# yangdongchao/Text-to-sound-Synthesis

Measured on NVIDIA H100. Metric: clips/sec (10s audio, 100 diffusion steps), higher is better.
Workload: dtype f16x3

## Files before the change

include/diffsound_b200.h:

```cpp
#ifndef DIFFSOUND_B200_H
#define DIFFSOUND_B200_H

#include <stdint.h>

#ifdef __cplusplus
extern "C" {
#endif

#define DSB_VERSION 100

#define DSB_DTYPE_TF32 0
#define DSB_DTYPE_BF16 1
#define DSB_DTYPE_F16 2

#define DSB_GEMM_GELU2 1
#define DSB_GEMM_ROUND_TF32 2
#define DSB_GEMM_OUT_BF16 4
#define DSB_GEMM_LRELU 8
#define DSB_GEMM_TANH 16
#define DSB_GEMM_OUT_F16 256
#define DSB_GEMM_RES_BEFORE_ACT 128
#define DSB_GEMM_DUAL_LRELU 4096
#define DSB_GEMM_NO_STORE 16384
#define DSB_GEMM_OUT_F16_SPLIT 2048
// ... 22 lines not shown
  int num_taps;
  int tap_shift[32];
  int tap_acol[32];
  long long a_cols;
  int geo_P, geo_Wp, geo_y0, geo_y1, geo_x0, geo_x1;
  float alpha;
  int block_n;
  int max_ctas;
  int cta_pair;
  int a_mn_major;
  int b_mn_major;
  int use_tap_wcol;
  int tap_wcol[32];
  long long w_cols;
  long long split_off;
  long long dual_off;
  int out_col_group;
  int out_col_group_stride;
  const void* A2;
  long long a2_rows, a2_cols, lda2, a2_batch_stride;
  int tap_a2[32];
  float* amax_out;
  int resident_w;
} dsb_gemm_desc;
int dsb_gemm_ex(const dsb_gemm_desc* desc, void* stream);

int dsb_gemm_f32(const float* A, const float* W, const float* bias, const float* residual, float* out, int M, int N, int K,
                 long long lda, long long ldw, long long ldo, long long ld_res, int flags, void* stream);

int dsb_round_tf32(const float* in, float* out, long long n, void* stream);
int dsb_f32_to_bf16(const float* in, void* out_bf16, long long n, void* stream);
int dsb_f32_to_f16(const float* in, void* out_f16, long long n, void* stream);
int dsb_split_f16(const float* in, long long ld_in, void* out_f16, long long ld_out, long long lo_off, long long rows, int C, float scale,
                  void* stream);
int dsb_split_tf32(const float* in, long long ld_in, float* out, long long ld_out, long long rows, int C, int Cp, int w_format, void* stream);

int dsb_embed_tokens(const int64_t* ids, const float* emb, const float* height_emb, const float* width_emb, float* out, int B, int L,
                     int D, int H, int W, int num_embed, int* err_flag, void* stream);

int dsb_layernorm(const float* x, void* out, const float* gamma, const float* beta, int rows, int D, float eps, int flags, void* stream);

int dsb_ada_layernorm(const float* x, void* out, const float* table, const int64_t* t, int B, int L, int D, int T, float eps, int flags,
                      void* stream);

int dsb_l2_normalize_rows(float* x, long long rows, int D, void* stream);

// ... 87 lines not shown
```

text-to-sound-synthesis_b200/_lib.py:

```python
from __future__ import annotations

import ctypes as C
import os

_HERE = os.path.dirname(os.path.abspath(__file__))
LIB_PATH = os.path.join(_HERE, "libdiffsound_b200.so")

c_vp, c_i, c_ll, c_f = C.c_void_p, C.c_int, C.c_longlong, C.c_float


class GemmDesc(C.Structure):
    _fields_ = [
        ("A", c_vp), ("W", c_vp), ("bias", c_vp), ("residual", c_vp), ("out", c_vp),
        ("M", c_i), ("N", c_i), ("K", c_i), ("batch", c_i),
        ("a_rows", c_ll), ("lda", c_ll), ("ldw", c_ll), ("ldo", c_ll), ("ld_res", c_ll),
        ("a_batch_stride", c_ll), ("w_batch_stride", c_ll), ("out_batch_stride", c_ll), ("res_batch_stride", c_ll),
        ("dtype", c_i), ("flags", c_i), ("num_taps", c_i), ("tap_shift", c_i * 32), ("tap_acol", c_i * 32), ("a_cols", c_ll),
        ("geo_P", c_i), ("geo_Wp", c_i), ("geo_y0", c_i), ("geo_y1", c_i), ("geo_x0", c_i), ("geo_x1", c_i),
        ("alpha", c_f), ("block_n", c_i), ("max_ctas", c_i), ("cta_pair", c_i), ("a_mn_major", c_i), ("b_mn_major", c_i),
        ("use_tap_wcol", c_i), ("tap_wcol", c_i * 32), ("w_cols", c_ll), ("split_off", c_ll),
        ("dual_off", c_ll), ("out_col_group", c_i), ("out_col_group_stride", c_i), ("A2", c_vp),
        ("a2_rows", c_ll), ("a2_cols", c_ll), ("lda2", c_ll), ("a2_batch_stride", c_ll), ("tap_a2", c_i * 32), ("amax_out", c_vp), ("resident_w", c_i),
    ]


SIGNATURES = {
    "dsb_version": [],
    "dsb_device_info": [C.POINTER(c_i)] * 3,
    "dsb_gemm_ex": [C.POINTER(GemmDesc), c_vp],
    "dsb_gemm_f32": [c_vp] * 5 + [c_i] * 3 + [c_ll] * 4 + [c_i, c_vp],
    "dsb_round_tf32": [c_vp, c_vp, c_ll, c_vp],
    "dsb_f32_to_bf16": [c_vp, c_vp, c_ll, c_vp],
    "dsb_f32_to_f16": [c_vp, c_vp, c_ll, c_vp],
    "dsb_silu": [c_vp, c_vp, c_ll, c_vp],
    "dsb_split_f16": [c_vp, c_ll, c_vp, c_ll, c_ll, c_ll, c_i, c_f, c_vp],
    "dsb_attention_tc_split": [c_vp, c_ll, c_ll, c_vp, c_ll, c_ll, c_vp, c_ll, c_ll, c_vp, c_ll, c_ll, c_i, c_i, c_i, c_i, c_f, c_vp],
    "dsb_l2_normalize_rows": [c_vp, c_ll, c_i, c_vp],
    "dsb_split_tf32": [c_vp, c_ll, c_vp, c_ll, c_ll, c_i, c_i, c_i, c_vp],
    "dsb_embed_tokens": [c_vp] * 5 + [c_i] * 6 + [c_vp, c_vp],
    "dsb_layernorm": [c_vp] * 4 + [c_i, c_i, c_f, c_i, c_vp],
    "dsb_ada_layernorm": [c_vp] * 4 + [c_i] * 4 + [c_f, c_i, c_vp],
    "dsb_attention": [c_vp, c_ll, c_vp, c_ll, c_vp, c_ll, c_vp, c_ll, c_i, c_i, c_i, c_i, c_f, c_i, c_vp],
    "dsb_codebook_gather_padded": [c_vp] * 3 + [c_i] * 6 + [c_vp, c_vp],
    "dsb_groupnorm_stats": [c_vp, c_vp] + [c_i] * 4 + [c_vp],
    "dsb_groupnorm_apply": [c_vp] * 5 + [c_i] * 5 + [c_f, c_i, c_i, c_vp],
# ... 60 lines not shown
```

text-to-sound-synthesis_b200/csrc/common.cuh:

```cuda
#pragma once
#include <cuda_runtime.h>
#include <cuda.h>
#include <cstdint>
#include <cstdio>

namespace dsb {

void set_error(const char* fmt, ...);
#define DSB_CHECK_CUDA(expr)                                                                    \
  do {                                                                                          \
    cudaError_t _e = (expr);                                                                    \
    if (_e != cudaSuccess) {                                                                    \
      dsb::set_error("%s:%d: %s -> %s", __FILE__, __LINE__, #expr, cudaGetErrorString(_e));     \
      return 1;                                                                                 \
    }                                                                                           \
  } while (0)
#define DSB_REQUIRE(cond, ...)                                                                  \
  do {                                                                                          \
    if (!(cond)) {                                                                              \
      dsb::set_error(__VA_ARGS__);                                                              \
      return 2;                                                                                 \
    }                                                                                           \
  } while (0)

// ... 59 lines not shown
__device__ __forceinline__ bool mbar_try_wait(uint64_t* bar, uint32_t parity) {
  uint32_t ok;
  asm volatile(
      "{\n\t.reg .pred P;\n\t"
      "mbarrier.try_wait.parity.shared::cta.b64 P, [%1], %2;\n\t"
      "selp.u32 %0, 1, 0, P;\n\t}"
      : "=r"(ok)
      : "r"(smem_u32(bar)), "r"(parity)
      : "memory");
  return ok != 0;
}
__device__ __forceinline__ void mbar_wait(uint64_t* bar, uint32_t parity) {
  uint32_t spins = 0;
  while (!mbar_try_wait(bar, parity)) {
    if (++spins > (1u << 26)) {
#ifdef DSB_MBAR_DEBUG
      printf("dsb: mbarrier wait timeout (block %d thread %d)\n", blockIdx.x, threadIdx.x);
#endif
      __trap();
    }
  }
}

__device__ __forceinline__ void prefetch_tmap(const CUtensorMap* m) {
  asm volatile("prefetch.tensormap [%0];" ::"l"(reinterpret_cast<uint64_t>(m)) : "memory");
}
__device__ __forceinline__ void tma_load_3d(const CUtensorMap* m, uint64_t* bar, void* dst, int c0, int c1, int c2) {
  asm volatile(
      "cp.async.bulk.tensor.3d.shared::cluster.global.mbarrier::complete_tx::bytes [%0], [%1, {%3, %4, %5}], [%2];"
      ::"r"(smem_u32(dst)), "l"(reinterpret_cast<uint64_t>(m)), "r"(smem_u32(bar)), "r"(c0), "r"(c1), "r"(c2)
      : "memory");
}

__device__ __forceinline__ void wgmma_fence() { asm volatile("wgmma.fence.sync.aligned;" ::: "memory"); }
__device__ __forceinline__ void wgmma_commit() { asm volatile("wgmma.commit_group.sync.aligned;" ::: "memory"); }
template <int N>
__device__ __forceinline__ void wgmma_wait() { asm volatile("wgmma.wait_group.sync.aligned %0;" ::"n"(N) : "memory"); }
template <int N>
__device__ __forceinline__ void wgmma_fence_regs(float (&d)[N]) {
#pragma unroll
  for (int i = 0; i < N; ++i) asm volatile("" : "+f"(d[i])::"memory");
}
template <uint32_t R>
__device__ __forceinline__ void setmaxnreg_inc() { asm volatile("setmaxnreg.inc.sync.aligned.u32 %0;" ::"n"(R)); }
template <uint32_t R>
__device__ __forceinline__ void setmaxnreg_dec() { asm volatile("setmaxnreg.dec.sync.aligned.u32 %0;" ::"n"(R)); }
// ... 13 lines not shown
```

text-to-sound-synthesis_b200/csrc/gemm_wgmma.cu:

```cuda
#include "common.cuh"
#include "diffsound_b200.h"
#include "wgmma.cuh"
#include <cuda_bf16.h>
#include <cuda_fp16.h>
#include <cstdlib>
#include <type_traits>

namespace dsb {

constexpr int BLOCK_M = 128;
constexpr int ROW_BYTES = 128;
constexpr int GEMM_THREADS = 384;
constexpr int MAX_TAPS = 32;
constexpr int MN_BOX_BYTES = 64 * ROW_BYTES;
constexpr int EPI_ROWS = 16;
constexpr int SMEM_BUDGET = 192 * 1024;

struct GemmParams {
  int M, N, batch;
  int tiles_m, tiles_n;
  int kb_per_tap;
  int block_k;
  int num_taps;
  int tap_shift[MAX_TAPS];
  int tap_acol[MAX_TAPS];
  int tap_wcol[MAX_TAPS];
  unsigned tap_a2_mask;
  int f3_nsp, lo_a, lo_w;
  long long split_off;
  long long dual_off;
  int ocg, ocg_stride;
  float* amax_out;
  int kc;
  int b_batched;
  const float* bias;
  const float* residual;
  long long ld_res, res_bstride;
  void* out;
  long long ldo, out_bstride;
  int flags;
  int geo_P, geo_Wp, geo_y0, geo_y1, geo_x0, geo_x1;
  float alpha;
  int a_mn, b_mn;
};

template <int BLOCK_N, bool F3>
struct GemmSmem {
  static constexpr int A_BYTES = BLOCK_M * ROW_BYTES;
  static constexpr int B_BYTES = BLOCK_N * ROW_BYTES;
  static constexpr int STAGE_BYTES = (F3 ? 2 : 1) * (A_BYTES + B_BYTES);
  static constexpr int STAGES = SMEM_BUDGET / STAGE_BYTES;
  static constexpr int EPI_BYTES = 8 * EPI_ROWS * 32 * 4;
  static constexpr int TOTAL = STAGES * STAGE_BYTES + EPI_BYTES + 256  + 1024 ;
};

__device__ __forceinline__ void epilogue_chunk(const GemmParams& p, const float* sw, int row_base, int col0, int b, int lane, bool vec_ok) {
  const bool has_geo = p.geo_P > 0;
  const int out_mode = (p.flags & DSB_GEMM_OUT_F16_SPLIT) ? 3 : ((p.flags & DSB_GEMM_OUT_F16) ? 1 : ((p.flags & DSB_GEMM_OUT_BF16) ? 2 : 0));
  const int act = (p.flags & DSB_GEMM_GELU2) ? 1 : ((p.flags & DSB_GEMM_LRELU) ? 2 : ((p.flags & DSB_GEMM_TANH) ? 3 : 0));
  const bool do_round = (p.flags & DSB_GEMM_ROUND_TF32) != 0;
  const bool dual = (p.flags & DSB_GEMM_DUAL_LRELU) != 0;
  const bool res_first = (p.flags & DSB_GEMM_RES_BEFORE_ACT) != 0;
  const int c4 = lane & 7;
  const int rsub = lane >> 3;
  constexpr int NI = EPI_ROWS / 4;
  uint32_t ok_mask = 0, in_mask = 0;
#pragma unroll
// ... 183 lines not shown
      }
    }
  }
}

template <int BLOCK_N, int KIND, bool F3>
__global__ void __launch_bounds__(GEMM_THREADS, 1)
gemm_wgmma_kernel(const __grid_constant__ CUtensorMap tmap_a, const __grid_constant__ CUtensorMap tmap_a2, const __grid_constant__ CUtensorMap tmap_b,
                  const __grid_constant__ GemmParams p) {
  using S = GemmSmem<BLOCK_N, F3>;
  constexpr int STAGES = S::STAGES;
  constexpr int NH = BLOCK_N / 128;
  static_assert(!F3 || NH == 1, "the split-fp16 form runs 128-wide tiles");
  extern __shared__ uint8_t smem_raw[];
  uint8_t* smem = reinterpret_cast<uint8_t*>((reinterpret_cast<uintptr_t>(smem_raw) + 1023) & ~uintptr_t(1023));
  float* epi_smem = reinterpret_cast<float*>(smem + STAGES * S::STAGE_BYTES);
  uint64_t* full_bar = reinterpret_cast<uint64_t*>(smem + STAGES * S::STAGE_BYTES + S::EPI_BYTES);
  uint64_t* empty_bar = full_bar + STAGES;

  const int warp = threadIdx.x >> 5;
  const int lane = threadIdx.x & 31;
  const int num_tiles = p.tiles_m * p.tiles_n * p.batch;
  const int num_kb = F3 ? p.kb_per_tap * p.f3_nsp : p.kb_per_tap * p.num_taps;

  if (threadIdx.x == 0) {
    prefetch_tmap(&tmap_a);
    prefetch_tmap(&tmap_a2);
    prefetch_tmap(&tmap_b);
    for (int s = 0; s < STAGES; ++s) {
      mbar_init(&full_bar[s], 1);
      mbar_init(&empty_bar[s], 8);
    }
    fence_barrier_init();
  }
  __syncthreads();
  pdl_wait();
  pdl_trigger();

  if (warp < 4) {
    setmaxnreg_dec<40>();
    if (threadIdx.x == 0) {
      int stage = 0;
      uint32_t phase = 0;
      for (int tile = blockIdx.x; tile < num_tiles; tile += gridDim.x) {
        const int m_blk = tile % p.tiles_m;
        const int n_blk = (tile / p.tiles_m) % p.tiles_n;
        const int b = tile / (p.tiles_m * p.tiles_n);
        for (int kb = 0; kb < num_kb; ++kb) {
          const int tap = kb / p.kb_per_tap;
          const int c0 = (kb - tap * p.kb_per_tap) * p.block_k;
          mbar_wait(&empty_bar[stage], phase ^ 1);
          mbar_arrive_expect_tx(&full_bar[stage], S::STAGE_BYTES);
          uint8_t* sa = smem + stage * S::STAGE_BYTES;
          if constexpr (F3) {
            const int arow = m_blk * BLOCK_M + p.tap_shift[tap], acol = p.tap_acol[tap] + c0, wcol = p.tap_wcol[tap] + c0;
            tma_load_3d(&tmap_a, &full_bar[stage], sa, acol, arow, b);
            tma_load_3d(&tmap_a, &full_bar[stage], sa + S::A_BYTES, acol + p.lo_a, arow, b);
            tma_load_3d(&tmap_b, &full_bar[stage], sa + 2 * S::A_BYTES, wcol, n_blk * BLOCK_N, 0);
            tma_load_3d(&tmap_b, &full_bar[stage], sa + 2 * S::A_BYTES + S::B_BYTES, wcol + p.lo_w, n_blk * BLOCK_N, 0);
          } else {
            if (p.a_mn) {
#pragma unroll
              for (int j = 0; j < BLOCK_M / 64; ++j) tma_load_3d(&tmap_a, &full_bar[stage], sa + j * MN_BOX_BYTES, m_blk * BLOCK_M + j * 64, c0, b);
            } else {
              tma_load_3d(((p.tap_a2_mask >> tap) & 1u) ? &tmap_a2 : &tmap_a, &full_bar[stage], sa, c0 + p.tap_acol[tap], m_blk * BLOCK_M + p.tap_shift[tap], b);
            }
            if (p.b_mn) {
#pragma unroll
              for (int j = 0; j < BLOCK_N / 64; ++j)
                tma_load_3d(&tmap_b, &full_bar[stage], sa + S::A_BYTES + j * MN_BOX_BYTES, n_blk * BLOCK_N + j * 64, c0, p.b_batched ? b : 0);
            } else {
              tma_load_3d(&tmap_b, &full_bar[stage], sa + S::A_BYTES, p.tap_wcol[tap] + c0, n_blk * BLOCK_N, p.b_batched ? b : 0);
            }
          }
          if (++stage == STAGES) { stage = 0; phase ^= 1; }
        }
      }
    }
  } else {
    setmaxnreg_inc<232>();
    const int wg = (warp >> 2) - 1;
    const int wq = warp & 3;
    float* sw = epi_smem + (warp - 4) * (EPI_ROWS * 32);
    const bool vec_ok = ((p.ldo & 3) == 0) && ((p.out_bstride & 3) == 0) && ((p.split_off & 3) == 0) && ((p.dual_off & 3) == 0) && ((p.ocg & 3) == 0) &&
                        ((p.ocg_stride & 3) == 0) &&
                        ((reinterpret_cast<uintptr_t>(p.out) & (4 * ((p.flags & (DSB_GEMM_OUT_F16_SPLIT | DSB_GEMM_OUT_F16 | DSB_GEMM_OUT_BF16)) ? 2 : 4) - 1)) == 0) &&
                        (!p.residual || (((p.ld_res & 3) == 0) && ((p.res_bstride & 3) == 0) && ((reinterpret_cast<uintptr_t>(p.residual) & 15) == 0))) &&
                        (!p.bias || ((reinterpret_cast<uintptr_t>(p.bias) & 15) == 0));
    int stage = 0;
    uint32_t phase = 0;
    for (int tile = blockIdx.x; tile < num_tiles; tile += gridDim.x) {
      const int m_blk = tile % p.tiles_m;
      const int n_blk = (tile / p.tiles_m) % p.tiles_n;
      const int b = tile / (p.tiles_m * p.tiles_n);
      float acc[NH][64];
#pragma unroll
      for (int h = 0; h < NH; ++h)
#pragma unroll
        for (int i = 0; i < 64; ++i) acc[h][i] = 0.f;
      int prev_stage = -1;
      if constexpr (F3) {
        float part[64];
        for (int kb = 0; kb < num_kb; ++kb) {
          mbar_wait(&full_bar[stage], phase);
          const uint32_t sa = smem_u32(smem + stage * S::STAGE_BYTES);
          wgmma_fence_regs(part);
          wgmma_fence();
          float(&pp)[1][64] = *reinterpret_cast<float(*)[1][64]>(&part);
          mma_kblock<KIND, 0, 0, 1, true>(pp, sa, wg, 0);
          wgmma_commit();
          wgmma_wait<0>();
          wgmma_fence_regs(part);
          if (lane == 0) mbar_arrive(&empty_bar[stage]);
#pragma unroll
          for (int i = 0; i < 64; ++i) acc[0][i] += part[i];
          if (++stage == STAGES) { stage = 0; phase ^= 1; }
        }
      } else {
        auto mainloop = [&](auto ta, auto tb) {
          for (int kb = 0; kb < num_kb; ++kb) {
            mbar_wait(&full_bar[stage], phase);
            const uint32_t sa = smem_u32(smem + stage * S::STAGE_BYTES);
#pragma unroll
            for (int h = 0; h < NH; ++h) wgmma_fence_regs(acc[h]);
            wgmma_fence();
            mma_kblock<KIND, decltype(ta)::value, decltype(tb)::value, NH, false>(acc, sa, wg, kb);
            wgmma_commit();
#pragma unroll
            for (int h = 0; h < NH; ++h) wgmma_fence_regs(acc[h]);
            wgmma_wait<1>();
            if (prev_stage >= 0 && lane == 0) mbar_arrive(&empty_bar[prev_stage]);
            prev_stage = stage;
            if (++stage == STAGES) { stage = 0; phase ^= 1; }
          }
        };
        using K0 = std::integral_constant<int, 0>;
        using K1 = std::integral_constant<int, 1>;
        if constexpr (KIND == DSB_DTYPE_TF32) mainloop(K0{}, K0{});
        else if (!p.a_mn && !p.b_mn) mainloop(K0{}, K0{});
        else if (p.a_mn && !p.b_mn) mainloop(K1{}, K0{});
        else if (!p.a_mn) mainloop(K0{}, K1{});
        else mainloop(K1{}, K1{});
      }
      wgmma_wait<0>();
#pragma unroll
      for (int h = 0; h < NH; ++h) wgmma_fence_regs(acc[h]);
      if (prev_stage >= 0 && lane == 0) mbar_arrive(&empty_bar[prev_stage]);

      const int row_base = m_blk * BLOCK_M + wg * 64 + wq * 16;
      const int n_chunks = min(BLOCK_N / 32, (p.N - n_blk * BLOCK_N + 31) / 32);
      const int r0 = lane >> 2, cc = 2 * (lane & 3);
#pragma unroll
      for (int c = 0; c < BLOCK_N / 32; ++c) {
        if (c < n_chunks) {
          const int h = c >> 2, j0 = (c & 3) * 4;
#pragma unroll
          for (int jj = 0; jj < 4; ++jj) {
            const int col = 8 * jj + cc;
            *reinterpret_cast<float2*>(sw + r0 * 32 + (((col >> 2) ^ (r0 & 7)) << 2) + (col & 3)) =
                make_float2(acc[h][4 * (j0 + jj)], acc[h][4 * (j0 + jj) + 1]);
            *reinterpret_cast<float2*>(sw + (r0 + 8) * 32 + (((col >> 2) ^ ((r0 + 8) & 7)) << 2) + (col & 3)) =
                make_float2(acc[h][4 * (j0 + jj) + 2], acc[h][4 * (j0 + jj) + 3]);
          }
          __syncwarp();
          epilogue_chunk(p, sw, row_base, n_blk * BLOCK_N + c * 32, b, lane, vec_ok);
          __syncwarp();
        }
      }
    }
  }
// ... 32 lines not shown
  DSB_REQUIRE(r == CUDA_SUCCESS, "cuTensorMapEncodeTiled failed (%d): k=%lld rows=%lld batch=%lld ld=%lld", (int)r, kdim, rows, batch, ld_elems);
  return 0;
}

int make_operand_map_mn(CUtensorMap* map, const void* ptr, int kind, long long mn, long long krows, long long batch, long long ld_elems,
                        long long bstride_elems) {
  PFN_encodeTiled enc = get_encode();
  DSB_REQUIRE(enc != nullptr, "cuTensorMapEncodeTiled entry point unavailable (no CUDA driver?)");
  DSB_REQUIRE(kind != DSB_DTYPE_TF32, "MN-major GEMM operands are implemented for the 2-byte types only");
  DSB_REQUIRE((reinterpret_cast<uintptr_t>(ptr) & 15) == 0, "GEMM operand pointer must be 16-byte aligned");
  DSB_REQUIRE((ld_elems * 2) % 16 == 0, "GEMM operand leading dimension must be a multiple of 16 bytes (ld=%lld)", ld_elems);
  DSB_REQUIRE(batch == 1 || (bstride_elems * 2) % 16 == 0, "GEMM batch stride must be a multiple of 16 bytes");
  cuuint64_t gdim[3] = {(cuuint64_t)mn, (cuuint64_t)krows, (cuuint64_t)batch};
  cuuint64_t gstr[2] = {(cuuint64_t)(ld_elems * 2), (cuuint64_t)((batch == 1 ? ld_elems * krows : bstride_elems) * 2)};
  cuuint32_t box[3] = {64, 64, 1};
  cuuint32_t estr[3] = {1, 1, 1};
  CUresult r = enc(map, kind == DSB_DTYPE_BF16 ? CU_TENSOR_MAP_DATA_TYPE_BFLOAT16 : CU_TENSOR_MAP_DATA_TYPE_FLOAT16, 3, const_cast<void*>(ptr), gdim, gstr,
                   box, estr, CU_TENSOR_MAP_INTERLEAVE_NONE, CU_TENSOR_MAP_SWIZZLE_128B, CU_TENSOR_MAP_L2_PROMOTION_L2_256B,
                   CU_TENSOR_MAP_FLOAT_OOB_FILL_NONE);
  DSB_REQUIRE(r == CUDA_SUCCESS, "cuTensorMapEncodeTiled (MN-major) failed (%d): mn=%lld k=%lld batch=%lld ld=%lld", (int)r, mn, krows, batch, ld_elems);
  return 0;
}

template <int BLOCK_N, int KIND, bool F3>
static int launch(const CUtensorMap& ma, const CUtensorMap& ma2, const CUtensorMap& mb, const GemmParams& p, int max_ctas, cudaStream_t st) {
  using S = GemmSmem<BLOCK_N, F3>;
  auto kern = gemm_wgmma_kernel<BLOCK_N, KIND, F3>;
  static bool attr_done = false;
  if (!attr_done) {
    DSB_CHECK_CUDA(cudaFuncSetAttribute(kern, cudaFuncAttributeMaxDynamicSharedMemorySize, S::TOTAL));
    attr_done = true;
  }
  const int tiles = p.tiles_m * p.tiles_n * p.batch;
  int grid = tiles < max_ctas ? tiles : max_ctas;
  DSB_CHECK_CUDA(launch_pdl(kern, dim3(grid), dim3(GEMM_THREADS), S::TOTAL, st, ma, ma2, mb, p));
  return 0;
}

}

using namespace dsb;

extern "C" int dsb_gemm_ex(const dsb_gemm_desc* d, void* stream) {
  DSB_REQUIRE(d != nullptr, "dsb_gemm_ex: null descriptor");
  DSB_REQUIRE(d->M > 0 && d->N > 0 && d->K > 0 && d->batch > 0, "dsb_gemm_ex: bad shape M=%d N=%d K=%d batch=%d", d->M, d->N, d->K, d->batch);
  DSB_REQUIRE(d->num_taps >= 1 && d->num_taps <= MAX_TAPS, "dsb_gemm_ex: num_taps=%d out of range", d->num_taps);
  DSB_REQUIRE(d->dtype == DSB_DTYPE_TF32 || d->dtype == DSB_DTYPE_BF16 || d->dtype == DSB_DTYPE_F16,
              "dsb_gemm_ex: dtype must be TF32, BF16 or F16 (use dsb_gemm_f32 for exact fp32)");
  const int kind = d->dtype;
  const int block_k = kind == DSB_DTYPE_TF32 ? 32 : 64;
  GemmParams p{};
  p.M = d->M; p.N = d->N; p.batch = d->batch;
  p.tiles_m = (d->M + BLOCK_M - 1) / BLOCK_M;
  p.kb_per_tap = (d->K + block_k - 1) / block_k;
  p.block_k = block_k;
  p.num_taps = d->num_taps;
  for (int i = 0; i < MAX_TAPS; ++i) {
// ... 16 lines not shown
    for (int i = 0; i < d->num_taps; ++i)
      if (d->tap_a2[i]) p.tap_a2_mask |= 1u << i;
  }
  DSB_REQUIRE(!(d->flags & DSB_GEMM_DUAL_LRELU) || ((d->flags & DSB_GEMM_OUT_F16_SPLIT) && d->dual_off > 0),
              "dsb_gemm_ex: DSB_GEMM_DUAL_LRELU needs DSB_GEMM_OUT_F16_SPLIT and dual_off > 0");
  DSB_REQUIRE(d->out_col_group == 0 || ((d->flags & DSB_GEMM_OUT_F16_SPLIT) && d->out_col_group % 4 == 0 && d->out_col_group_stride % 4 == 0 && !d->residual),
              "dsb_gemm_ex: output column groups need the split-fp16 output, multiples of 4 and no residual");
  p.kc = d->K;
  p.b_batched = d->w_batch_stride != 0;
  p.bias = d->bias; p.residual = d->residual; p.ld_res = d->ld_res; p.res_bstride = d->res_batch_stride;
  p.out = d->out; p.ldo = d->ldo; p.out_bstride = d->out_batch_stride;
  p.flags = d->flags;
  p.geo_P = d->geo_P; p.geo_Wp = d->geo_Wp; p.geo_y0 = d->geo_y0; p.geo_y1 = d->geo_y1; p.geo_x0 = d->geo_x0; p.geo_x1 = d->geo_x1;
  p.alpha = d->alpha == 0.0f ? 1.0f : d->alpha;
  p.a_mn = d->a_mn_major != 0;
  p.b_mn = d->b_mn_major != 0;
  const bool any_mn = p.a_mn || p.b_mn;
  DSB_REQUIRE(!any_mn || (kind != DSB_DTYPE_TF32 && d->num_taps == 1 && d->tap_shift[0] == 0 && d->tap_acol[0] == 0),
              "dsb_gemm_ex: MN-major operands need a 2-byte dtype and a single unshifted tap");
  if (d->resident_w)
    DSB_REQUIRE(kind != DSB_DTYPE_TF32 && !any_mn && !p.b_batched && d->K == 64 && d->N <= 128 && d->use_tap_wcol,
                "dsb_gemm_ex: resident_w needs a 2-byte dtype, K-major operands, K == 64 per tap, N <= 128, explicit tap_wcol and an unbatched W");
  DSB_REQUIRE(!(any_mn && d->cta_pair > 0), "dsb_gemm_ex: 256 x 256 pair tiles take K-major operands only");

  const int sms = sm_count();
  const int max_ctas = d->max_ctas > 0 ? d->max_ctas : sms;
  int block_n = d->block_n;
  if (block_n == 0 && d->cta_pair > 0) block_n = 256;
  if (block_n == 0) {
    if (d->N <= 128) block_n = 128;
    else {
      const long long t256 = (long long)p.tiles_m * ((d->N + 255) / 256) * d->batch;
      const long long t128 = (long long)p.tiles_m * ((d->N + 127) / 128) * d->batch;
      const long long cost256 = ((t256 + sms - 1) / sms) * 2, cost128 = ((t128 + sms - 1) / sms);
      block_n = cost128 < cost256 ? 128 : 256;
    }
  }
  DSB_REQUIRE(block_n == 128 || block_n == 256, "dsb_gemm_ex: block_n must be 0, 128 or 256");
  bool fused3 = kind == DSB_DTYPE_F16 && d->cta_pair >= 0 && d->num_taps % 3 == 0 && !p.tap_a2_mask && !p.b_batched && !any_mn && d->K % 64 == 0;
  int f3_lo_a = 0, f3_lo_w = 0;
  if (fused3) {
    f3_lo_a = p.tap_acol[0] - p.tap_acol[1];
    f3_lo_w = p.tap_wcol[1] - p.tap_wcol[0];
    for (int j = 0; j < d->num_taps && fused3; j += 3)
      fused3 = p.tap_shift[j] == p.tap_shift[j + 1] && p.tap_shift[j] == p.tap_shift[j + 2] && p.tap_acol[j + 1] == p.tap_acol[j + 2] &&
               p.tap_acol[j] - p.tap_acol[j + 1] == f3_lo_a && p.tap_wcol[j] == p.tap_wcol[j + 2] && p.tap_wcol[j + 1] - p.tap_wcol[j] == f3_lo_w;
// ... 5 lines not shown
  CUtensorMap ma, mb;
  const long long a_rows = d->a_rows > 0 ? d->a_rows : d->M;
  if (p.a_mn) {
    if (make_operand_map_mn(&ma, d->A, kind, a_rows, d->K, d->batch, d->lda, d->a_batch_stride)) return 3;
  } else if (make_operand_map(&ma, d->A, kind, d->a_cols > 0 ? d->a_cols : d->K, a_rows, d->batch, d->lda, d->a_batch_stride, BLOCK_M)) return 3;
  if (p.b_mn) {
    if (make_operand_map_mn(&mb, d->W, kind, d->N, d->K, p.b_batched ? d->batch : 1, d->ldw, d->w_batch_stride)) return 3;
  } else if (make_operand_map(&mb, d->W, kind, d->w_cols > 0 ? d->w_cols : (long long)d->K * d->num_taps, d->N, p.b_batched ? d->batch : 1, d->ldw,
                              d->w_batch_stride, block_n)) return 3;
  CUtensorMap ma2 = ma;
  if (p.tap_a2_mask) {
    DSB_REQUIRE(!any_mn, "dsb_gemm_ex: a second A operand is K-major only");
    if (make_operand_map(&ma2, d->A2, kind, d->a2_cols > 0 ? d->a2_cols : d->K, d->a2_rows > 0 ? d->a2_rows : d->M, d->batch, d->lda2, d->a2_batch_stride, BLOCK_M)) return 3;
  }
  cudaStream_t st = reinterpret_cast<cudaStream_t>(stream);
  if (fused3) {
    p.f3_nsp = d->num_taps / 3;
    p.lo_a = f3_lo_a;
    p.lo_w = f3_lo_w;
    for (int j = 0; j < p.f3_nsp; ++j) {
      const int sh = p.tap_shift[3 * j], ac = p.tap_acol[3 * j + 1], wc = p.tap_wcol[3 * j];
      p.tap_shift[j] = sh; p.tap_acol[j] = ac; p.tap_wcol[j] = wc;
    }
    return launch<128, DSB_DTYPE_F16, true>(ma, ma2, mb, p, max_ctas, st);
  }
  if (block_n == 256) {
    if (kind == DSB_DTYPE_TF32) return launch<256, DSB_DTYPE_TF32, false>(ma, ma2, mb, p, max_ctas, st);
    if (kind == DSB_DTYPE_BF16) return launch<256, DSB_DTYPE_BF16, false>(ma, ma2, mb, p, max_ctas, st);
    return launch<256, DSB_DTYPE_F16, false>(ma, ma2, mb, p, max_ctas, st);
  }
  if (kind == DSB_DTYPE_TF32) return launch<128, DSB_DTYPE_TF32, false>(ma, ma2, mb, p, max_ctas, st);
  if (kind == DSB_DTYPE_BF16) return launch<128, DSB_DTYPE_BF16, false>(ma, ma2, mb, p, max_ctas, st);
  return launch<128, DSB_DTYPE_F16, false>(ma, ma2, mb, p, max_ctas, st);
}
```

text-to-sound-synthesis_b200/ops.py:

```python
from __future__ import annotations

import ctypes as C
from typing import Optional, Sequence

import torch

from . import _lib

TF32, BF16, F16 = 0, 1, 2
GELU2, ROUND_TF32, OUT_BF16, LRELU, TANH, GN_SWISH, GN_COMPACT, RES_BEFORE_ACT, OUT_F16, SPLIT_OUT = 1, 2, 4, 8, 16, 32, 64, 128, 256, 512
OUT_F16_SPLIT = 2048
DUAL_LRELU = 4096
SPLIT_OUT_F16 = 8192
NO_STORE = 16384


def _stream() -> int:
    return torch.cuda.current_stream().cuda_stream


def _ptr(t: Optional[torch.Tensor]):
    return None if t is None else t.data_ptr()


# ... 88 lines not shown
    if w_pair.shape[-1] != 2 * K:
        raise RuntimeError(f"gemm_f16x3: W pair has {w_pair.shape[-1]} columns, expected {2 * K}")
    N = w_pair.shape[0]
    M = a_pair.shape[0]
    if out is None:
        out = torch.empty(M, 2 * N, dtype=torch.float16, device=a_pair.device) if split_out else torch.empty(M, N, dtype=torch.float32, device=a_pair.device)
    return gemm(a_pair, w_pair, bias, residual, out, dtype=F16, taps=[0, 0, 0], tap_acol=[K, 0, 0], tap_wcol=[0, K, 0], k_per_tap=K, alpha=alpha,
                gelu=gelu, split_out=split_out, **kw)


def silu(x: torch.Tensor, out: Optional[torch.Tensor] = None) -> torch.Tensor:
    _need_cuda(x, out)
    x = x.contiguous()
    out = torch.empty_like(x) if out is None else out
    _lib.check(_lib.lib().dsb_silu(x.data_ptr(), out.data_ptr(), x.numel(), _stream()), "dsb_silu")
    return out


def gemm(a: torch.Tensor, w: torch.Tensor, bias: Optional[torch.Tensor] = None, residual: Optional[torch.Tensor] = None,
         out: Optional[torch.Tensor] = None, *, dtype: int = TF32, gelu: bool = False, round_out: bool = False, out_bf16: bool = False, out_f16: bool = False,
         lrelu: bool = False, tanh: bool = False, res_before_act: bool = False, taps: Optional[Sequence[int]] = None,
         tap_acol: Optional[Sequence[int]] = None, k_per_tap: Optional[int] = None, out_rows: Optional[int] = None, geo: Optional[Sequence[int]] = None, alpha: float = 1.0,
         block_n: int = 0, max_ctas: int = 0, cta_pair: int = 0, a_mn: bool = False, w_mn: bool = False,
         tap_wcol: Optional[Sequence[int]] = None, split_out: bool = False) -> torch.Tensor:
    _need_cuda(a, w, bias, residual, out)
    batched = a.dim() == 3
    if a.stride(-1) != 1 or w.stride(-1) != 1:
        raise RuntimeError("gemm operands must be contiguous in their last dimension")
    ntaps = 1 if taps is None else len(taps)
    batch = a.shape[0] if batched else 1
    a_rows, a_cols = (a.shape[-1], a.shape[-2]) if a_mn else (a.shape[-2], a.shape[-1])
    K = a_cols if k_per_tap is None else k_per_tap
    N = w.shape[-1] if w_mn else w.shape[-2]
    if tap_wcol is None and (w.shape[-2] if w_mn else w.shape[-1]) != K * ntaps:
        raise RuntimeError(f"gemm: W has reduction length {w.shape[-2] if w_mn else w.shape[-1]}, expected {K}*{ntaps}")
    M = a_rows if out_rows is None else out_rows
    odt = torch.bfloat16 if out_bf16 else (torch.float16 if out_f16 else torch.float32)
    if out is None:
        out = torch.empty((batch, M, N) if batched else (M, N), dtype=odt, device=a.device)
    out_f16 = out.dtype == torch.float16 and not split_out
    out_bf16 = out.dtype == torch.bfloat16
    if split_out and (out.dtype != torch.float16 or batched):
        raise RuntimeError("gemm: split_out writes an fp16 (hi | lo) pair and is not batched")
    d = _lib.GemmDesc()
    d.A, d.W, d.bias, d.residual, d.out = a.data_ptr(), w.data_ptr(), _ptr(bias), _ptr(residual), out.data_ptr()
    d.M, d.N, d.K, d.batch = M, N, K, batch
    d.a_rows = a_rows
# ... 2 lines not shown
    d.a_batch_stride = a.stride(0) if batched else 0
    d.w_batch_stride = w.stride(0) if w.dim() == 3 else 0
    d.out_batch_stride = out.stride(0) if batched else 0
    d.res_batch_stride = residual.stride(0) if (residual is not None and batched) else 0
    d.dtype = dtype
    d.flags = (GELU2 if gelu else 0) | (ROUND_TF32 if round_out else 0) | (OUT_BF16 if out_bf16 else 0) | (LRELU if lrelu else 0) | (TANH if tanh else 0) | (RES_BEFORE_ACT if res_before_act else 0) | (OUT_F16 if out_f16 else 0) | (OUT_F16_SPLIT if split_out else 0)
    if split_out:
        d.split_off = N
    if tap_wcol is not None:
        d.use_tap_wcol = 1
        d.w_cols = w.shape[-1]
        for i, c_ in enumerate(tap_wcol):
            d.tap_wcol[i] = int(c_)
    d.num_taps = ntaps
    for i, s in enumerate(taps or [0]):
        d.tap_shift[i] = int(s)
        d.tap_acol[i] = int(tap_acol[i]) if tap_acol is not None else 0
    d.a_cols = a_cols
    if geo is not None:
        d.geo_P, d.geo_Wp, d.geo_y0, d.geo_y1, d.geo_x0, d.geo_x1 = [int(v) for v in geo]
    d.alpha = alpha
    d.block_n, d.max_ctas, d.cta_pair = block_n, max_ctas, cta_pair
    d.a_mn_major, d.b_mn_major = int(a_mn), int(w_mn)
    _lib.check(_lib.lib().dsb_gemm_ex(C.byref(d), _stream()), "dsb_gemm_ex")
    return out


def gemm_desc(*, A, W, out, M, N, K, taps, lda, ldw, ldo, dtype=F16, batch=1, a_rows=0, a_cols=0, a_batch_stride=0, w_cols=0, out_batch_stride=0,
              bias=None, flags=0, alpha=1.0, split_off=0, dual_off=0, out_col_group=0, out_col_group_stride=0, A2=None, lda2=0, a2_rows=0, a2_cols=0,
              a2_batch_stride=0, block_n=0, cta_pair=0, residual=None, ld_res=0, geo=None, amax_out=None, resident_w=0):
    d = _lib.GemmDesc()
    d.A, d.W, d.out, d.bias, d.A2 = A, W, out, _ptr(bias), A2
    d.M, d.N, d.K, d.batch = M, N, K, batch
    d.a_rows, d.a_cols, d.lda, d.ldw, d.ldo = a_rows, a_cols, lda, ldw, ldo
    d.a_batch_stride, d.out_batch_stride = a_batch_stride, out_batch_stride
    d.dtype, d.flags, d.alpha = dtype, flags, alpha
    d.num_taps = len(taps)
    d.use_tap_wcol, d.w_cols = 1, w_cols
    for i, (sh, ac, wc, a2) in enumerate(taps):
        d.tap_shift[i], d.tap_acol[i], d.tap_wcol[i], d.tap_a2[i] = int(sh), int(ac), int(wc), int(a2)
    d.split_off, d.dual_off, d.out_col_group, d.out_col_group_stride = split_off, dual_off, out_col_group, out_col_group_stride
    d.lda2, d.a2_rows, d.a2_cols, d.a2_batch_stride = lda2, a2_rows, a2_cols, a2_batch_stride
    d.block_n, d.cta_pair = block_n, cta_pair
    d.residual, d.ld_res = residual, ld_res
    d.amax_out = _ptr(amax_out)
    d.resident_w = int(resident_w)
    if geo is not None:
        d.geo_P, d.geo_Wp, d.geo_y0, d.geo_y1, d.geo_x0, d.geo_x1 = [int(v) for v in geo]
    _lib.check(_lib.lib().dsb_gemm_ex(C.byref(d), _stream()), "dsb_gemm_ex")


def mel_pack_f16(mel, pad, Kp):
    _need_cuda(mel)
    B, Cm, T = mel.shape
    out = torch.empty(B, T + 2 * pad, 2 * Kp, dtype=torch.float16, device=mel.device)
    _lib.check(_lib.lib().dsb_mel_pack_f16(mel.data_ptr(), out.data_ptr(), B, Cm, T, pad, Kp, _stream()), "dsb_mel_pack_f16")
    return out


def edge_pad_f16(state, T, P, d, col0, ncols, reflect=True):
    _need_cuda(state)
    B, Tp, ld = state.shape
    _lib.check(_lib.lib().dsb_edge_pad_f16(state.data_ptr(), ld, Tp * ld, B, T, P, d, col0, ncols, 1 if reflect else 0, _stream()), "dsb_edge_pad_f16")


def conv_out_pair(state, T, row0, col0, w, bias, scale, out=None):
    _need_cuda(state, w, bias)
    B, rows, ld = state.shape
    kt, cs = w.shape
# ... 251 lines not shown
```

Measured before the change: 8.056.

## Add stream-K scheduling to the WGMMA GEMM for partial-wave tile counts

Adds a stream-K work split to the persistent WGMMA GEMM. When the tile count is between one and three waves and not a multiple of the grid, the last tiles are split along K across CTAs. Each partial tile hands its fp32 accumulators to the next CTA through a global workspace, using acquire/release flags. The goal is to remove wave-quantization idle time on the last wave, at the cost of spin-waiting, extra global traffic for partial sums, and a workspace that is lazily allocated per device and skipped under graph capture.

```diff
diff --git a/include/diffsound_b200.h b/include/diffsound_b200.h
--- a/include/diffsound_b200.h
+++ b/include/diffsound_b200.h
@@ -68,6 +68,7 @@
   int tap_a2[32];
   float* amax_out;
   int resident_w;
+  int schedule;
 } dsb_gemm_desc;
 int dsb_gemm_ex(const dsb_gemm_desc* desc, void* stream);
 
diff --git a/text-to-sound-synthesis_b200/_lib.py b/text-to-sound-synthesis_b200/_lib.py
--- a/text-to-sound-synthesis_b200/_lib.py
+++ b/text-to-sound-synthesis_b200/_lib.py
@@ -21,6 +21,7 @@
         ("use_tap_wcol", c_i), ("tap_wcol", c_i * 32), ("w_cols", c_ll), ("split_off", c_ll),
         ("dual_off", c_ll), ("out_col_group", c_i), ("out_col_group_stride", c_i), ("A2", c_vp),
         ("a2_rows", c_ll), ("a2_cols", c_ll), ("lda2", c_ll), ("a2_batch_stride", c_ll), ("tap_a2", c_i * 32), ("amax_out", c_vp), ("resident_w", c_i),
+        ("schedule", c_i),
     ]
 
 
diff --git a/text-to-sound-synthesis_b200/csrc/common.cuh b/text-to-sound-synthesis_b200/csrc/common.cuh
--- a/text-to-sound-synthesis_b200/csrc/common.cuh
+++ b/text-to-sound-synthesis_b200/csrc/common.cuh
@@ -105,6 +105,14 @@
   }
 }
 
+__device__ __forceinline__ int ld_acquire_gpu(const int* p) {
+  int v;
+  asm volatile("ld.acquire.gpu.global.b32 %0, [%1];" : "=r"(v) : "l"(p) : "memory");
+  return v;
+}
+__device__ __forceinline__ void st_release_gpu(int* p, int v) { asm volatile("st.release.gpu.global.b32 [%0], %1;" ::"l"(p), "r"(v) : "memory"); }
+__device__ __forceinline__ void named_bar_sync(int id, int threads) { asm volatile("bar.sync %0, %1;" ::"r"(id), "r"(threads) : "memory"); }
+
 __device__ __forceinline__ void prefetch_tmap(const CUtensorMap* m) {
   asm volatile("prefetch.tensormap [%0];" ::"l"(reinterpret_cast<uint64_t>(m)) : "memory");
 }
diff --git a/text-to-sound-synthesis_b200/csrc/gemm_wgmma.cu b/text-to-sound-synthesis_b200/csrc/gemm_wgmma.cu
--- a/text-to-sound-synthesis_b200/csrc/gemm_wgmma.cu
+++ b/text-to-sound-synthesis_b200/csrc/gemm_wgmma.cu
@@ -1,9 +1,11 @@
 #include "common.cuh"
 #include "diffsound_b200.h"
+#include "stream_k.cuh"
 #include "wgmma.cuh"
 #include <cuda_bf16.h>
 #include <cuda_fp16.h>
 #include <cstdlib>
+#include <mutex>
 #include <type_traits>
 
 namespace dsb {
@@ -42,7 +44,13 @@
   int geo_P, geo_Wp, geo_y0, geo_y1, geo_x0, geo_x1;
   float alpha;
   int a_mn, b_mn;
+  int stream_k;
+  float* sk_part;
+  int* sk_flag;
 };
+
+constexpr int SK_SLOT_FLOATS = 128 * 128;
+constexpr unsigned SK_SPIN_LIMIT = 1u << 24;
 
 template <int BLOCK_N, bool F3>
 struct GemmSmem {
@@ -272,6 +280,8 @@
   const int lane = threadIdx.x & 31;
   const int num_tiles = p.tiles_m * p.tiles_n * p.batch;
   const int num_kb = F3 ? p.kb_per_tap * p.f3_nsp : p.kb_per_tap * p.num_taps;
+  const dsb_sk::Work work = dsb_sk::cta_work(num_tiles, num_kb, gridDim.x, blockIdx.x, p.stream_k != 0);
+  const int n_pieces = dsb_sk::num_pieces(work);
 
   if (threadIdx.x == 0) {
     prefetch_tmap(&tmap_a);
@@ -292,11 +302,12 @@
     if (threadIdx.x == 0) {
       int stage = 0;
       uint32_t phase = 0;
-      for (int tile = blockIdx.x; tile < num_tiles; tile += gridDim.x) {
-        const int m_blk = tile % p.tiles_m;
-        const int n_blk = (tile / p.tiles_m) % p.tiles_n;
-        const int b = tile / (p.tiles_m * p.tiles_n);
-        for (int kb = 0; kb < num_kb; ++kb) {
+      for (int pi = 0; pi < n_pieces; ++pi) {
+        const dsb_sk::Piece pc = dsb_sk::piece(work, num_kb, pi);
+        const int m_blk = pc.tile % p.tiles_m;
+        const int n_blk = (pc.tile / p.tiles_m) % p.tiles_n;
+        const int b = pc.tile / (p.tiles_m * p.tiles_n);
+        for (int kb = pc.kb0; kb < pc.kb1; ++kb) {
           const int tap = kb / p.kb_per_tap;
           const int c0 = (kb - tap * p.kb_per_tap) * p.block_k;
           mbar_wait(&empty_bar[stage], phase ^ 1);
@@ -337,21 +348,42 @@
                         ((reinterpret_cast<uintptr_t>(p.out) & (4 * ((p.flags & (DSB_GEMM_OUT_F16_SPLIT | DSB_GEMM_OUT_F16 | DSB_GEMM_OUT_BF16)) ? 2 : 4) - 1)) == 0) &&
                         (!p.residual || (((p.ld_res & 3) == 0) && ((p.res_bstride & 3) == 0) && ((reinterpret_cast<uintptr_t>(p.residual) & 15) == 0))) &&
                         (!p.bias || ((reinterpret_cast<uintptr_t>(p.bias) & 15) == 0));
+    const int ct = threadIdx.x - 128;
     int stage = 0;
     uint32_t phase = 0;
-    for (int tile = blockIdx.x; tile < num_tiles; tile += gridDim.x) {
-      const int m_blk = tile % p.tiles_m;
-      const int n_blk = (tile / p.tiles_m) % p.tiles_n;
-      const int b = tile / (p.tiles_m * p.tiles_n);
+    for (int pi = 0; pi < n_pieces; ++pi) {
+      const dsb_sk::Piece pc = dsb_sk::piece(work, num_kb, pi);
+      const int m_blk = pc.tile % p.tiles_m;
+      const int n_blk = (pc.tile / p.tiles_m) % p.tiles_n;
+      const int b = pc.tile / (p.tiles_m * p.tiles_n);
       float acc[NH][64];
-#pragma unroll
-      for (int h = 0; h < NH; ++h)
-#pragma unroll
-        for (int i = 0; i < 64; ++i) acc[h][i] = 0.f;
+      const bool tail = pc.kb0 > 0;
+      if (tail) {
+        if (ct == 0) {
+          int* flag = p.sk_flag + blockIdx.x - 1;
+          unsigned spins = 0;
+          while (ld_acquire_gpu(flag) == 0) {
+            if (++spins > SK_SPIN_LIMIT) __trap();
+            __nanosleep(64);
+          }
+          *flag = 0;
+        }
+        named_bar_sync(1, 256);
+      }
+      {
+        const float4* slot = reinterpret_cast<const float4*>(p.sk_part + (size_t)(blockIdx.x - 1) * NH * SK_SLOT_FLOATS);
+#pragma unroll
+        for (int h = 0; h < NH; ++h)
+#pragma unroll
+          for (int q = 0; q < 16; ++q) {
+            const float4 v = tail ? __ldcg(slot + (h * 16 + q) * 256 + ct) : make_float4(0.f, 0.f, 0.f, 0.f);
+            acc[h][4 * q] = v.x; acc[h][4 * q + 1] = v.y; acc[h][4 * q + 2] = v.z; acc[h][4 * q + 3] = v.w;
+          }
+      }
       int prev_stage = -1;
       if constexpr (F3) {
         float part[64];
-        for (int kb = 0; kb < num_kb; ++kb) {
+        for (int kb = pc.kb0; kb < pc.kb1; ++kb) {
           mbar_wait(&full_bar[stage], phase);
           const uint32_t sa = smem_u32(smem + stage * S::STAGE_BYTES);
           wgmma_fence_regs(part);
@@ -368,7 +400,7 @@
         }
       } else {
         auto mainloop = [&](auto ta, auto tb) {
-          for (int kb = 0; kb < num_kb; ++kb) {
+          for (int kb = pc.kb0; kb < pc.kb1; ++kb) {
             mbar_wait(&full_bar[stage], phase);
             const uint32_t sa = smem_u32(smem + stage * S::STAGE_BYTES);
 #pragma unroll
@@ -396,6 +428,18 @@
 #pragma unroll
       for (int h = 0; h < NH; ++h) wgmma_fence_regs(acc[h]);
       if (prev_stage >= 0 && lane == 0) mbar_arrive(&empty_bar[prev_stage]);
+
+      if (pc.kb1 < num_kb) {
+        float4* slot = reinterpret_cast<float4*>(p.sk_part + (size_t)blockIdx.x * NH * SK_SLOT_FLOATS);
+#pragma unroll
+        for (int h = 0; h < NH; ++h)
+#pragma unroll
+          for (int q = 0; q < 16; ++q) __stcg(slot + (h * 16 + q) * 256 + ct, make_float4(acc[h][4 * q], acc[h][4 * q + 1], acc[h][4 * q + 2], acc[h][4 * q + 3]));
+        __threadfence();
+        named_bar_sync(1, 256);
+        if (ct == 0) st_release_gpu(p.sk_flag + blockIdx.x, 1);
+        continue;
+      }
 
       const int row_base = m_blk * BLOCK_M + wg * 64 + wq * 16;
       const int n_chunks = min(BLOCK_N / 32, (p.N - n_blk * BLOCK_N + 31) / 32);
@@ -474,8 +518,30 @@
   return 0;
 }
 
+static int sk_workspace(cudaStream_t st, float** part, int** flag) {
+  static std::mutex mu;
+  static void* ws[64] = {};
+  int dev = 0;
+  DSB_CHECK_CUDA(cudaGetDevice(&dev));
+  DSB_REQUIRE(dev < 64, "dsb_gemm_ex: device %d out of range for the stream-K workspace", dev);
+  std::lock_guard<std::mutex> lock(mu);
+  if (!ws[dev]) {
+    cudaStreamCaptureStatus cap = cudaStreamCaptureStatusNone;
+    DSB_CHECK_CUDA(cudaStreamIsCapturing(st, &cap));
+    if (cap != cudaStreamCaptureStatusNone) return 0;
+    const size_t bytes = (size_t)sm_count() * (2 * SK_SLOT_FLOATS * sizeof(float) + sizeof(int));
+    void* w = nullptr;
+    DSB_CHECK_CUDA(cudaMalloc(&w, bytes));
+    DSB_CHECK_CUDA(cudaMemsetAsync(w, 0, bytes, st));
+    ws[dev] = w;
+  }
+  *part = static_cast<float*>(ws[dev]);
+  *flag = reinterpret_cast<int*>(*part + (size_t)sm_count() * 2 * SK_SLOT_FLOATS);
+  return 0;
+}
+
 template <int BLOCK_N, int KIND, bool F3>
-static int launch(const CUtensorMap& ma, const CUtensorMap& ma2, const CUtensorMap& mb, const GemmParams& p, int max_ctas, cudaStream_t st) {
+static int launch(const CUtensorMap& ma, const CUtensorMap& ma2, const CUtensorMap& mb, GemmParams& p, int max_ctas, int schedule, cudaStream_t st) {
   using S = GemmSmem<BLOCK_N, F3>;
   auto kern = gemm_wgmma_kernel<BLOCK_N, KIND, F3>;
   static bool attr_done = false;
@@ -485,6 +551,12 @@
   }
   const int tiles = p.tiles_m * p.tiles_n * p.batch;
   int grid = tiles < max_ctas ? tiles : max_ctas;
+  const int num_kb = F3 ? p.kb_per_tap * p.f3_nsp : p.kb_per_tap * p.num_taps;
+  p.stream_k = 0;
+  if (schedule == 0 && dsb_sk::stream_k_applies(tiles, num_kb, grid, sm_count())) {
+    if (int r = sk_workspace(st, &p.sk_part, &p.sk_flag)) return r;
+    p.stream_k = p.sk_part != nullptr;
+  }
   DSB_CHECK_CUDA(launch_pdl(kern, dim3(grid), dim3(GEMM_THREADS), S::TOTAL, st, ma, ma2, mb, p));
   return 0;
 }
@@ -547,6 +619,7 @@
     DSB_REQUIRE(kind != DSB_DTYPE_TF32 && !any_mn && !p.b_batched && d->K == 64 && d->N <= 128 && d->use_tap_wcol,
                 "dsb_gemm_ex: resident_w needs a 2-byte dtype, K-major operands, K == 64 per tap, N <= 128, explicit tap_wcol and an unbatched W");
   DSB_REQUIRE(!(any_mn && d->cta_pair > 0), "dsb_gemm_ex: 256 x 256 pair tiles take K-major operands only");
+  DSB_REQUIRE(d->schedule == 0 || d->schedule == 1, "dsb_gemm_ex: schedule must be 0 (auto) or 1 (data-parallel only)");
 
   const int sms = sm_count();
   const int max_ctas = d->max_ctas > 0 ? d->max_ctas : sms;
@@ -598,14 +671,14 @@
       const int sh = p.tap_shift[3 * j], ac = p.tap_acol[3 * j + 1], wc = p.tap_wcol[3 * j];
       p.tap_shift[j] = sh; p.tap_acol[j] = ac; p.tap_wcol[j] = wc;
     }
-    return launch<128, DSB_DTYPE_F16, true>(ma, ma2, mb, p, max_ctas, st);
+    return launch<128, DSB_DTYPE_F16, true>(ma, ma2, mb, p, max_ctas, d->schedule, st);
   }
   if (block_n == 256) {
-    if (kind == DSB_DTYPE_TF32) return launch<256, DSB_DTYPE_TF32, false>(ma, ma2, mb, p, max_ctas, st);
-    if (kind == DSB_DTYPE_BF16) return launch<256, DSB_DTYPE_BF16, false>(ma, ma2, mb, p, max_ctas, st);
-    return launch<256, DSB_DTYPE_F16, false>(ma, ma2, mb, p, max_ctas, st);
-  }
-  if (kind == DSB_DTYPE_TF32) return launch<128, DSB_DTYPE_TF32, false>(ma, ma2, mb, p, max_ctas, st);
-  if (kind == DSB_DTYPE_BF16) return launch<128, DSB_DTYPE_BF16, false>(ma, ma2, mb, p, max_ctas, st);
-  return launch<128, DSB_DTYPE_F16, false>(ma, ma2, mb, p, max_ctas, st);
-}
+    if (kind == DSB_DTYPE_TF32) return launch<256, DSB_DTYPE_TF32, false>(ma, ma2, mb, p, max_ctas, d->schedule, st);
+    if (kind == DSB_DTYPE_BF16) return launch<256, DSB_DTYPE_BF16, false>(ma, ma2, mb, p, max_ctas, d->schedule, st);
+    return launch<256, DSB_DTYPE_F16, false>(ma, ma2, mb, p, max_ctas, d->schedule, st);
+  }
+  if (kind == DSB_DTYPE_TF32) return launch<128, DSB_DTYPE_TF32, false>(ma, ma2, mb, p, max_ctas, d->schedule, st);
+  if (kind == DSB_DTYPE_BF16) return launch<128, DSB_DTYPE_BF16, false>(ma, ma2, mb, p, max_ctas, d->schedule, st);
+  return launch<128, DSB_DTYPE_F16, false>(ma, ma2, mb, p, max_ctas, d->schedule, st);
+}
diff --git a/text-to-sound-synthesis_b200/csrc/stream_k.cuh b/text-to-sound-synthesis_b200/csrc/stream_k.cuh
--- /dev/null
+++ b/text-to-sound-synthesis_b200/csrc/stream_k.cuh
@@ -0,0 +1,63 @@
+#pragma once
+
+#ifdef __CUDACC__
+#define DSB_SK __host__ __device__ __forceinline__
+#else
+#define DSB_SK inline
+#endif
+
+namespace dsb_sk {
+
+struct Piece {
+  int tile, kb0, kb1;
+};
+
+struct Work {
+  int head_tile, head_kb;
+  int dp0, dp_step, n_dp;
+  int tile0, n_whole;
+  int tail_tile, tail_kb;
+};
+
+DSB_SK bool stream_k_applies(int num_tiles, int num_kb, int grid, int sms) {
+  return grid <= sms && num_tiles > grid && num_tiles < 3 * grid && num_tiles % grid != 0 && num_kb > 1 &&
+         (long long)num_tiles * num_kb <= 0x7fffffff;
+}
+
+DSB_SK Work cta_work(int num_tiles, int num_kb, int grid, int c, bool stream_k) {
+  Work w{};
+  w.dp0 = c;
+  w.dp_step = grid;
+  if (!stream_k) {
+    w.n_dp = c < num_tiles ? (num_tiles - c + grid - 1) / grid : 0;
+    return w;
+  }
+  const int sk_tiles = grid + num_tiles % grid, dp_tiles = num_tiles - sk_tiles;
+  w.n_dp = dp_tiles / grid;
+  const int units = sk_tiles * num_kb, q = units / grid, r = units % grid;
+  const int u0 = q * c + r * c / grid, u1 = q * (c + 1) + r * (c + 1) / grid;
+  const int t0 = dp_tiles + u0 / num_kb, k0 = u0 % num_kb;
+  const int t1 = dp_tiles + u1 / num_kb, k1 = u1 % num_kb;
+  w.tail_tile = t0;
+  w.tail_kb = k0;
+  w.tile0 = k0 > 0 ? t0 + 1 : t0;
+  w.n_whole = t1 - w.tile0;
+  w.head_tile = t1;
+  w.head_kb = k1;
+  return w;
+}
+
+DSB_SK int num_pieces(const Work& w) { return (w.head_kb > 0) + w.n_dp + w.n_whole + (w.tail_kb > 0); }
+
+DSB_SK Piece piece(const Work& w, int num_kb, int i) {
+  if (w.head_kb > 0) {
+    if (i == 0) return Piece{w.head_tile, 0, w.head_kb};
+    --i;
+  }
+  if (i < w.n_dp) return Piece{w.dp0 + i * w.dp_step, 0, num_kb};
+  i -= w.n_dp;
+  if (i < w.n_whole) return Piece{w.tile0 + i, 0, num_kb};
+  return Piece{w.tail_tile, w.tail_kb, num_kb};
+}
+
+}
diff --git a/text-to-sound-synthesis_b200/ops.py b/text-to-sound-synthesis_b200/ops.py
--- a/text-to-sound-synthesis_b200/ops.py
+++ b/text-to-sound-synthesis_b200/ops.py
@@ -134,7 +134,7 @@
          lrelu: bool = False, tanh: bool = False, res_before_act: bool = False, taps: Optional[Sequence[int]] = None,
          tap_acol: Optional[Sequence[int]] = None, k_per_tap: Optional[int] = None, out_rows: Optional[int] = None, geo: Optional[Sequence[int]] = None, alpha: float = 1.0,
          block_n: int = 0, max_ctas: int = 0, cta_pair: int = 0, a_mn: bool = False, w_mn: bool = False,
-         tap_wcol: Optional[Sequence[int]] = None, split_out: bool = False) -> torch.Tensor:
+         tap_wcol: Optional[Sequence[int]] = None, split_out: bool = False, schedule: int = 0) -> torch.Tensor:
     _need_cuda(a, w, bias, residual, out)
     batched = a.dim() == 3
     if a.stride(-1) != 1 or w.stride(-1) != 1:
@@ -183,13 +183,15 @@
     d.alpha = alpha
     d.block_n, d.max_ctas, d.cta_pair = block_n, max_ctas, cta_pair
     d.a_mn_major, d.b_mn_major = int(a_mn), int(w_mn)
+    d.schedule = schedule
     _lib.check(_lib.lib().dsb_gemm_ex(C.byref(d), _stream()), "dsb_gemm_ex")
     return out
 
 
 def gemm_desc(*, A, W, out, M, N, K, taps, lda, ldw, ldo, dtype=F16, batch=1, a_rows=0, a_cols=0, a_batch_stride=0, w_cols=0, out_batch_stride=0,
               bias=None, flags=0, alpha=1.0, split_off=0, dual_off=0, out_col_group=0, out_col_group_stride=0, A2=None, lda2=0, a2_rows=0, a2_cols=0,
-              a2_batch_stride=0, block_n=0, cta_pair=0, residual=None, ld_res=0, geo=None, amax_out=None, resident_w=0):
+              a2_batch_stride=0, block_n=0, cta_pair=0, residual=None, ld_res=0, geo=None, amax_out=None, resident_w=0,
+              schedule=0):
     d = _lib.GemmDesc()
     d.A, d.W, d.out, d.bias, d.A2 = A, W, out, _ptr(bias), A2
     d.M, d.N, d.K, d.batch = M, N, K, batch
@@ -206,6 +208,7 @@
     d.residual, d.ld_res = residual, ld_res
     d.amax_out = _ptr(amax_out)
     d.resident_w = int(resident_w)
+    d.schedule = schedule
     if geo is not None:
         d.geo_P, d.geo_Wp, d.geo_y0, d.geo_y1, d.geo_x0, d.geo_x1 = [int(v) for v in geo]
     _lib.check(_lib.lib().dsb_gemm_ex(C.byref(d), _stream()), "dsb_gemm_ex")
```

Result: faster. 8.318 (median of 6 runs) (+3.2%).
